# xinge008/SCDA

Hardware: AMD Instinct MI355X
Metric: images/sec (fwd+bwd) VGG16 Faster-RCNN+SCDA 512x1024 (higher is better)
Workload: dtype f32; 1 GPU; vgg16_FasterRCNN + 4-cluster SCDA, synthetic Cityscapes->Foggy 512x1024, batch=1/GPU (BASELINE.json configs[1]); 1 step = 1 source + 1 target image, 4 optimiser phases; gt_boxes=12, rois=512, clusters=4, recon=256, parallelism=dp1

## Files before the change

include/scda_ops.h:

```cpp
#ifndef SCDA_OPS_H
#define SCDA_OPS_H

#include <stddef.h>
#include <stdint.h>

#ifdef __cplusplus
extern "C" {
#endif

#define SCDA_OK 0
#define SCDA_EINVAL (-1)
#define SCDA_ELAUNCH (-2)
#define SCDA_ENODEV (-3)

int scda_version(void);
int scda_device_count(void);
const char *scda_last_error(void);

void scda_prof_enable(unsigned kernel_mask);
int scda_prof_num_kernels(void);
const char *scda_prof_kernel_name(int k);
int scda_prof_collect(long long *launches, double *ms, double *flops, double *bytes);
void scda_debug_last_plan(int *out4);
void scda_debug_plan_conv(int dir, int batch, int Cin, int IH, int IW, int Cout, int KH, int KW, int S, int P, int row_period,
// ... 142 lines not shown
size_t scda_eval_mark_duplicates_workspace_bytes(int n);
int scda_eval_mark_duplicates_hip(const int *image_ids, int n, void *ws, int *first, int *flags, int raise_on_duplicate, void *stream);
int scda_map_merge_duplicates_hip(const int *first, int n, int D, const int *box, const float *score, const int *cls, const int *rank,
                                  const int *kept, int *tp, int *flags, void *stream);

size_t scda_conv2d_workspace_bytes(int batch, int Cin, int IH, int IW, int Cout, int KH, int KW, int S, int P);
size_t scda_conv2d_packed_elems(int Cout, int Cin, int KH, int KW, int for_dgrad);
int scda_conv2d_pack_weight_hip(const float *w, float *out, int Cout, int Cin, int KH, int KW, int for_dgrad,
                                void *stream);
long long scda_conv2d_pack_tiles(int Cout, int Cin, int KH, int KW, int for_dgrad);
int scda_conv2d_pack_weights_batched_hip(const float *base, float *out, const long long *desc, int n, long long n_tiles,
                                         void *stream);
int scda_conv2d_fwd_hip(const float *x, const float *wp, const float *bias , float *y, int batch,
                        int Cin, int IH, int IW, int Cout, int KH, int KW, int S, int P, int row_period, int act, float slope,
                        void *ws, size_t ws_bytes, void *stream);
int scda_conv2d_dgrad_hip(const float *dy, const float *wt, float *dx, int batch, int Cin, int IH, int IW, int Cout,
                          int KH, int KW, int S, int P, int row_period, void *ws, size_t ws_bytes, void *stream);
int scda_conv2d_dgrad_act_hip(const float *dy, const float *wt, float *dx, int batch, int Cin, int IH, int IW, int Cout,
                              int KH, int KW, int S, int P, int row_period, const float *act_src, float act_slope, void *ws,
                              size_t ws_bytes, void *stream);
int scda_conv2d_dgrad_small_cin_hip(const float *dy, const float *w, float *dx, int batch, int Cin, int IH, int IW, int Cout,
                                    int KH, int KW, int S, int P, void *stream);
int scda_conv2d_wgrad_hip(const float *dy, const float *x, float *dw, int batch, int Cin, int IH, int IW, int Cout,
                          int KH, int KW, int S, int P, int row_period, int accumulate, void *ws, size_t ws_bytes, void *stream);
int scda_conv2d_wgrad_bias_fusable(int batch, int Cout, int OH, int OW, const float *dy);
int scda_conv2d_wgrad_bias_hip(const float *dy, const float *x, float *dw, float *db, int batch, int Cin, int IH, int IW,
                               int Cout, int KH, int KW, int S, int P, int row_period, int accumulate, int db_accumulate, void *ws,
                               size_t ws_bytes, void *stream);

int scda_conv2d_wino_supported(int batch, int C, int H, int W, int M);
// ... 120 lines not shown
```

scda_amd/autograd_ops.py:

```python
import os

import torch
from torch.autograd import Function

from . import native as N

ACT_NONE, ACT_RELU, ACT_LEAKY = N.ACT_NONE, N.ACT_RELU, N.ACT_LEAKY


from .probe import replay as _replay


def _c(t):
    return t if t.is_contiguous() else t.contiguous()


def _mask_src(ctx, y, kind="act"):
    r = _replay()
    if r is not None and any(ctx.needs_input_grad):
        return r.act(y)
    return y


def _sink(p):
# ... 40 lines not shown
            dw = None if sw is not None else dw
            db = None if sb is not None else db
        elif want_w:
            sink = _sink(ctx.w_ref)
            dw = N.conv2d_wgrad(dy, x, w.shape, stride, pad, out=sink, row_period=rp)
            if sink is not None:
                dw = None
        elif want_b:
            sink = _sink(ctx.bias_ref)
            db = N.bias_grad_nchw(dy, out=sink)
            if sink is not None:
                db = None
        return dx, dw, db, None, None, None, None, None, None


class ConvPoolFn(Function):

    @staticmethod
    def forward(ctx, x, w, b, slope, in_act):
        x = _c(x)
        if isinstance(w, torch.nn.Parameter):
            w._scda_wino_used = True
        y, idx = N.conv2d_wino_pool(x, N.conv2d_wino_pack(w, False), b, w.shape[0], ACT_RELU, slope)
        ctx.in_act = in_act
        ctx.has_bias = b is not None
        ctx.bias_ref, ctx.w_ref = b, w
        ctx.save_for_backward(x, w, idx, y)
        return y

    @staticmethod
# ... 435 lines not shown
class GlobalAvgPoolFn(Function):
    @staticmethod
    def forward(ctx, x):
        ctx.xshape = tuple(x.shape)
        return N.gap_fwd(_c(x))

    @staticmethod
    def backward(ctx, dy):
        return N.gap_bwd(_c(dy), ctx.xshape)


def conv2d(x, w, b=None, stride=1, padding=0, act=ACT_NONE, slope=0.01, fuse=(None, False), row_period=0):
    return Conv2dFn.apply(x, w, b, stride, padding, act, slope, fuse, row_period)


def linear(x, w, b=None, act=ACT_NONE, defer_act_bwd=False):
    return LinearFn.apply(x, w, b, act, defer_act_bwd)


def adversarial_loss(groups, scale=1.0):
    k = len(groups)
    return AdvLossFn.apply(scale, k, *[g[0] for g in groups], *[g[1] for g in groups], *[g[2] for g in groups])


def cross_entropy(logits, targets, ignore_index=-100):
    return SoftmaxCEFn.apply(logits, targets, ignore_index)


def smooth_l1_sum(pred, mask, target, sigma=3.0, scale=1.0):
    return SmoothL1Fn.apply(pred, mask, target, sigma, scale)
# ... 13 lines not shown
```

scda_amd/csrc/conv_gemm.hip:

```cpp
#include <stdio.h>
#include <stdlib.h>
#include <string.h>

#include "launch_plan.h"
#include "mfma_tile.h"
#include "wino_pack.h"

namespace scda {

__device__ __forceinline__ void tile_coords(const int nx, const int ny, const int swz, int &tx, int &ty, int &tz) {
    const unsigned nwg = gridDim.x, id = blockIdx.x;
    unsigned L = id;
    if (swz) {
        const unsigned q = nwg >> 3, r = nwg & 7, xcd = id & 7;
        L = (xcd < r ? xcd * (q + 1) : r * (q + 1) + (xcd - r) * q) + (id >> 3);
    }
    if (swz & 2) {
        const unsigned per = (unsigned)nx * ny, z = L / per, r = L - z * per;
        const unsigned grp = r / (8u * nx), first = grp * 8u, gsz = min((unsigned)ny - first, 8u), rr = r - grp * 8u * nx;
        tz = (int)z;
        tx = (int)(rr / gsz);
        ty = (int)(first + rr - (unsigned)tx * gsz);
        return;
    }
// ... 1552 lines not shown
#pragma unroll
        for (int kw = 0; kw < 3; ++kw) {
            const int iy = py + kh - 1, ix = px + kw - 1;
            const bool ok = iy >= 0 && iy < H && ix >= 0 && ix < W;
#pragma unroll
            for (int c = 0; c < CIN; ++c) v[(kh * 3 + kw) * CIN + c] = ok ? xi[((size_t)c * H + iy) * W + ix] : 0.f;
        }
    float *yo = y + ((size_t)img * Cout * H + py) * W + px;
    for (int m = 0; m < Cout; ++m) {
        const float *wm = wk + m * (9 * CIN);
        float a = 0.f;
#pragma unroll
        for (int k = 0; k < 9 * CIN; ++k) a = fmaf(wm[k], v[k], a);
        if (bias) a += bias[m];
        yo[(size_t)m * H * W] = apply_act(a, act, slope);
    }
}

template <int KH, int KW>
__global__ __launch_bounds__(256) void conv_dgrad_small_cin_kernel(const float *__restrict__ dY, const float *__restrict__ W,
                                                                   float *__restrict__ dX, const int batch, const int Cin,
                                                                   const int IH, const int IW, const int Cout, const int OH,
                                                                   const int OW, const int S, const int P) {
    extern __shared__ __attribute__((aligned(16))) float wl[];
    constexpr int R = KH * KW;
    for (int i = threadIdx.x; i < Cout * R * 4; i += blockDim.x) {
        const int m = i & 3, r = (i >> 2) % R, co = (i >> 2) / R;
        wl[i] = m < Cin ? W[((size_t)co * Cin + m) * R + r] : 0.f;
    }
    __syncthreads();
// ... 342 lines not shown
    if (d.family == lp::FAM_SMALL_CIN) {
        const dim3 grid((unsigned)cdiv(IW, 256), (unsigned)IH, (unsigned)batch);
        note_plan(d);
        prof_begin(PK_CONV_GATHER, 2.0 * Cout * (double)g.N * g.K, st);
        if (Cin == 1) hipLaunchKernelGGL((conv3x3_small_cin_fwd_kernel<1>), grid, dim3(256), 0, st, x, w, bias, y, IH, IW, Cout, act, slope);
        else if (Cin == 2) hipLaunchKernelGGL((conv3x3_small_cin_fwd_kernel<2>), grid, dim3(256), 0, st, x, w, bias, y, IH, IW, Cout, act, slope);
        else if (Cin == 3) hipLaunchKernelGGL((conv3x3_small_cin_fwd_kernel<3>), grid, dim3(256), 0, st, x, w, bias, y, IH, IW, Cout, act, slope);
        else hipLaunchKernelGGL((conv3x3_small_cin_fwd_kernel<4>), grid, dim3(256), 0, st, x, w, bias, y, IH, IW, Cout, act, slope);
        prof_end(st);
        return launch_status("conv3x3_small_cin_fwd_kernel");
    }
    Epi e{y, nullptr, bias, 0, act, slope, 1, 0, nullptr, 0.f};
    if (KH == 7 && KW == 7 && S == 2)
        return launch_conv<7, 7, 2, false>(d, w, x, g, e, (float *)ws, st);
    CONV_DISPATCH(launch_conv, , false > (d, w, x, g, e, (float *)ws, st))
}

SCDA_API int scda_conv2d_dgrad_hip(const float *dy, const float *wt, float *dx, int batch, int Cin, int IH, int IW,
                                   int Cout, int KH, int KW, int S, int P, int row_period, void *ws, size_t ws_bytes, void *stream) {
    return scda_conv2d_dgrad_act_hip(dy, wt, dx, batch, Cin, IH, IW, Cout, KH, KW, S, P, row_period, nullptr, 0.f, ws, ws_bytes, stream);
}

SCDA_API int scda_conv2d_dgrad_act_hip(const float *dy, const float *wt, float *dx, int batch, int Cin, int IH, int IW,
                                       int Cout, int KH, int KW, int S, int P, int row_period_arg, const float *act_src, float act_slope,
                                       void *ws, size_t ws_bytes, void *stream) {
    const int row_period = take_row_period("scda_conv2d_dgrad_hip", row_period_arg, IH, KH, KW, S, P);
    if (row_period < 0) return SCDA_EINVAL;
    if (!dy || !wt || !dx || batch <= 0) { set_error("scda_conv2d_dgrad_hip: bad arguments"); return SCDA_EINVAL; }
    const lp::ConvShape c{batch, Cin, IH, IW, Cout, KH, KW, S, P, row_period};
    const int OH = c.OH(), OW = c.OW();
// ... 177 lines not shown
```

scda_amd/csrc/launch_plan.h:

```cpp
#ifndef SCDA_LAUNCH_PLAN_H
#define SCDA_LAUNCH_PLAN_H

#include <stddef.h>
#include <stdio.h>
#include <stdlib.h>
#include <string.h>

#include <algorithm>
#include <vector>

namespace scda {
namespace lp {

constexpr int BK = 16;
constexpr int X9_BM = 256, X9_BN = 128;

static inline int cdiv(long long a, long long b) { return (int)((a + b - 1) / b); }
static inline int conv_out_dim(int in, int k, int s, int p) { return (in + 2 * p - k) / s + 1; }
static inline int conv_packed_mpad(int M) { return M <= 64 ? 64 : (M + 127) / 128 * 128; }

struct ForcedPlan { bool set; int bm, bn, splits; };
struct PlanEnv {
    ForcedPlan force;
    bool allow_bm64;
// ... 254 lines not shown
    d.nx = cdiv(N, d.bn); d.ny = cdiv(M, d.bm);
    d.swz = 1;
    if (d.parity) {
        d.nc = c.batch * (PH / 2) * (PW / 2);
        d.ncp = cdiv(d.nc, d.bn) * d.bn;
        d.nx = 4 * (d.ncp / d.bn);
        d.splits = fit_splits(std::max(1, std::min(plan.splits, (CB / BK) * taps)), M, N, ws_bytes);
    } else if (grouped_tile_order(d.nx, d.ny, M, K)) {
        d.swz |= 2;
    }
    d.grid = d.nx * d.ny * d.splits;
    d.reduce = d.splits > 1;
    return d;
}

static LaunchDecision decide_wgrad(const ConvShape &c, bool dy_aligned, bool aligned, bool fused_bias, size_t ws_bytes, int n_cu, const PlanEnv &env) {
    const int OH = c.OH(), OW = c.OW();
    const int M = c.Cout, N = c.Cin * c.KH * c.KW, K = c.batch * OH * OW;
    if (c.gemm_1x1() && !fused_bias && conv1x1_takes_x9(aligned, M, N, K, K, K, 0, 0, env)) return decide_gemm_x9(M, N, K, N, ws_bytes, n_cu, env);
    const bool small = M <= 64;
    const bool fits_2g = (long long)c.Cout * OH * OW * 4 < (1LL << 31) && (long long)c.Cin * c.IH * c.IW * 4 < (1LL << 31);
    const bool glds = dy_aligned && ((OH * OW) % BK) == 0 && fits_2g;
    TileRules r{};
    r.bm = small ? 64 : 128;
    r.allow64 = N <= 64; r.allow128 = !r.allow64; r.must_split = true; r.k_granule = 32;
    r.allow_bm256 = glds && r.allow128 && (M % 256) == 0;
    r.bn32 = (glds && M <= 32 && r.allow128) ? 128 : 0;
    LaunchPlan plan = plan_tiles(M, N, K, r, ws_bytes, env);
    if (r.bn32 && !env.force.set) plan.bm = 32;
    LaunchDecision d{};
// ... 181 lines not shown
```

scda_amd/dropin/_impl/rpn_head.py:

```python
import torch.nn as nn

from scda_amd import layers as L
from scda_amd.autograd_ops import ACT_RELU


class NaiveRpnHead(nn.Module):
    def __init__(self, inplanes, num_classes, num_anchors):
        super().__init__()
        self.num_classes = num_classes
        self.num_anchors = num_anchors
        self.conv3x3 = L.Conv2d(inplanes, 512, kernel_size=3, stride=1, padding=1, fused_act=ACT_RELU)
        self.relu3x3 = L.FusedAct("ReLU")
        self.conv_cls = L.Conv2d(512, num_anchors * num_classes, kernel_size=1, stride=1)
        self.conv_loc = L.Conv2d(512, num_anchors * 4, kernel_size=1, stride=1)

    def forward(self, x):
        hidden = self.relu3x3(self.conv3x3(x))
        return self.conv_cls(hidden), self.conv_loc(hidden)
```

scda_amd/dropin/models/faster_rcnn/faster_rcnn_adver_expansion_reweight_cluster.py:

```python
import functools
import logging

import os
import torch
import torch.nn as nn

from scda_amd import autograd_ops as A
from scda_amd import layers as L
from scda_amd import native as N
from scda_amd._timing import mark
from scda_amd.dropin.functions.anchor_target import compute_anchor_targets
from scda_amd.dropin.functions.mask import compute_cluster_targets
from scda_amd.dropin.functions.predict_bbox import compute_predicted_bboxes
from scda_amd.dropin.functions.proposal_target import compute_proposal_targets
from scda_amd.dropin.functions.rpn_proposal import compute_rpn_proposals
from scda_amd.dropin.models.faster_rcnn.common_net import (INSResBlock, LeakyReLUConv2d, LeakyReLUConvTranspose2d_2, LinUnsRes_cluster2,
                                                           LinUnsRes_cluster, ResDis_cluster, gaussian_weights_init, pair_decoder_upsamples)

logger = logging.getLogger('global')


def smooth_l1_loss_with_sigma(pred, targets, sigma=3.0):
    return A.smooth_l1_sum(pred, None, targets.contiguous(), sigma, 1.0)

# ... 31 lines not shown
    nhwc = rpn_pred_cls.detach().permute(0, 2, 3, 1).contiguous()
    prob = N.row_softmax(nhwc.view(-1, 2)).view_as(nhwc)
    return prob.permute(0, 3, 1, 2)


class FasterRCNN_AdEx(nn.Module):
    def __init__(self, gan_model_flag):
        super().__init__()

    def feature_extractor(self, x):
        raise NotImplementedError

    def rpn(self, x):
        raise NotImplementedError

    def rcnn(self, x, rois):
        raise NotImplementedError

    def _add_rpn_loss(self, compute_anchor_targets_fn, rpn_pred_cls, rpn_pred_loc):
        cls_targets, loc_targets, loc_masks, loc_normalizer = compute_anchor_targets_fn(rpn_pred_loc.size())
        logits = rpn_pred_cls.permute(0, 2, 3, 1).contiguous().view(-1, 2)
        flat_t = cls_targets.permute(0, 2, 3, 1).contiguous().view(-1)
        rpn_loss_cls = A.cross_entropy(logits, flat_t, ignore_index=-1)
        rpn_loss_loc = A.smooth_l1_sum(rpn_pred_loc, loc_masks, loc_targets, 3.0, 1.0 / loc_normalizer)
        acc = accuracy(logits, flat_t)[0]
        return rpn_loss_cls, rpn_loss_loc, acc

    def _add_rcnn_loss(self, rcnn_pred_cls, rcnn_pred_loc, cls_targets, loc_targets, loc_weights):
        rcnn_loss_cls = A.cross_entropy(rcnn_pred_cls, cls_targets)
        rcnn_loss_loc = A.smooth_l1_sum(rcnn_pred_loc, loc_weights, loc_targets, 3.0, 1.0 / cls_targets.shape[0])
        acc = accuracy(rcnn_pred_cls, cls_targets)[0]
# ... 87 lines not shown
            hook(losses)
            mark('det_backward_enqueued')
        clu_fea, clu_ctr = compute_cluster_targets(rois, x_fea, N_cluster=input['cluster_num'], threshold=input['threshold'])
        mark('src_cluster')
        side = input.get('_side_stream')
        main = torch.cuda.current_stream(dev) if side is not None else None

        def target_branch():
            with torch.no_grad():
                proposals_t = fn['rpn_proposal_fn'](*tgt_host())
                outputs['num_proposals_target'] = int(proposals_t.shape[0])
                rois_t_host = proposals_t[0:512, :5].contiguous()
                rois_t = N.upload(rois_t_host, dev)
                rois_t._scda_host = rois_t_host.numpy()
                assert rois_t.shape[1] == 5
                x_fea_t, _, _ = self.rcnn(feat_t, rois_t)
                return (x_fea_t,) + compute_cluster_targets(rois_t, x_fea_t, N_cluster=input['cluster_num'],
                                                            threshold=input['threshold'])

        if side is None:
            x_fea_t, clu_fea_t, clu_ctr_t = target_branch()
        else:
            side.wait_event(ev_backbones)
            with torch.cuda.stream(side):
                x_fea_t, clu_fea_t, clu_ctr_t = target_branch()
            main.wait_stream(side)
            for t in (x_fea_t, clu_fea_t):
                t.record_stream(main)
        assert feat_t.size() == feat.size(), "gan_features does not match the backbone"
        mark('target_branch')

# ... 30 lines not shown
    def __init__(self, params):
        super().__init__()
        ch, cin, n_layer = params['ch'], params['input_dim_a'], params['n_layer']
        self.model_A = self._make_net(ch, cin, n_layer - 1)
        self.model_A.apply(gaussian_weights_init)
        self.model_B = self._make_net(ch, cin, n_layer - 1)
        self.model_B.apply(gaussian_weights_init)
        L.plan_act_fusion(self.model_A, self.model_B)

    def _make_net(self, ch, input_dim, n_layer):
        seq = [LeakyReLUConv2d(input_dim, ch, kernel_size=3, stride=2, padding=1)]
        for _ in range(n_layer):
            seq.append(LeakyReLUConv2d(ch, ch * 2, kernel_size=3, stride=2, padding=1))
            ch *= 2
        seq.append(L.Conv2d(ch, 1, kernel_size=1, stride=1, padding=0))
        return nn.Sequential(*seq)

    def forward(self, x_aa, x_bb):
        a, b = _two_branches(self, lambda: self.model_A(x_aa), lambda: self.model_B(x_bb))
        return a.view(a.size(0), -1), b.view(b.size(0), -1)


class GAN_dis_AE_patch(nn.Module):

    def __init__(self, params=None):
        super().__init__()
        if params:
            self.n_in, self.n_out, clusters = params['n_in'], params['n_out'], params['cluster_num']
        else:
            self.n_in, self.n_out, clusters = 128, 256, 4
# ... 45 lines not shown
```

scda_amd/dropin/models/faster_rcnn/vgg_adver_expansion_cluster.py:

```python
import math

import torch.nn as nn

from scda_amd import layers as L
from scda_amd.autograd_ops import ACT_NONE, ACT_RELU
from scda_amd.dropin.extensions import RoIPool
from scda_amd.dropin.models.faster_rcnn.faster_rcnn_adver_expansion_reweight_cluster import FasterRCNN_AdEx
from scda_amd.dropin.models.head import NaiveRpnHead

__all__ = ['VGG', 'vgg16', 'vgg16_bn']

cfg = {
    'A': [64, 'M', 128, 'M', 256, 256, 'M', 512, 512, 'M', 512, 512, 'M'],
    'B': [64, 64, 'M', 128, 128, 'M', 256, 256, 'M', 512, 512, 'M', 512, 512, 'M'],
    'D': [64, 64, 'M', 128, 128, 'M', 256, 256, 256, 'M', 512, 512, 512, 'M', 512, 512, 512, 'M'],
    'E': [64, 64, 'M', 128, 128, 'M', 256, 256, 256, 256, 'M', 512, 512, 512, 512, 'M', 512, 512, 512, 512, 'M'],
}


def make_layers(plan, batch_norm=False):
    seq, cin = [], 3
    for v in plan:
        if v == 'M':
            seq.append(L.MaxPool2x2())
# ... 17 lines not shown
        self.roipooling = RoIPool(7, 7, 1.0 / cfg['anchor_stride'])
        self.classifier = nn.Sequential(
            L.Linear(512 * 7 * 7, 4096, fused_act=ACT_RELU), L.FusedAct("ReLU"), L.Dropout(),
            L.Linear(4096, 4096, fused_act=ACT_RELU), L.FusedAct("ReLU"), L.Dropout())
        self.fc_rcnn_cls = L.Linear(4096, cfg['num_classes'])
        self.fc_rcnn_loc = L.Linear(4096, cfg['num_classes'] * 4)
        L.plan_act_fusion(self.features, self.classifier)
        self._initialize_weights()

    def feature_extractor(self, x):
        return self.features(x)

    def rpn(self, x):
        return self.rpn_head(x)

    def rcnn(self, x, rois):
        assert rois.shape[1] == 5
        pooled = self.roipooling(x, rois)
        hook = getattr(self, '_head_grad_hook', None)
        if hook is not None and pooled.requires_grad:
            pooled.register_hook(lambda g: hook())
        x_fea = self.classifier(pooled.view(pooled.size(0), -1))
        return x_fea, self.fc_rcnn_cls(x_fea), self.fc_rcnn_loc(x_fea)

    def _initialize_weights(self):
        for m in self.modules():
            if isinstance(m, nn.Conv2d):
                fan = m.kernel_size[0] * m.kernel_size[1] * m.out_channels
                m.weight.data.normal_(0, math.sqrt(2. / fan))
                if m.bias is not None:
                    m.bias.data.zero_()
            elif isinstance(m, nn.BatchNorm2d):
                m.weight.data.fill_(1)
                m.bias.data.zero_()
            elif isinstance(m, nn.Linear):
                m.weight.data.normal_(0, 0.01)
                m.bias.data.zero_()
# ... 15 lines not shown
```

scda_amd/dropin/models/mask_rcnn/resnet.py:

```python
import math
import os

import torch
import torch.nn as nn

from scda_amd import autograd_ops as A
from scda_amd import layers as L
from scda_amd import native as N
from scda_amd.autograd_ops import ACT_NONE, ACT_RELU
from scda_amd.dropin.extensions._roi_align.modules.roi_align import RoIAlignAvg
from scda_amd.dropin.extensions import RoIPool
from scda_amd.dropin.models.faster_rcnn.faster_rcnn_adver_expansion_reweight_cluster import FasterRCNN_AdEx
from scda_amd.dropin.models.head import NaiveRpnHead

__all__ = ['ResNet', 'Bottleneck', 'resnet50', 'resnet101']


def _frozen(conv, bn):
    return (not bn.training and not conv.weight.requires_grad and not bn.weight.requires_grad and bn.running_mean is not None
            and conv.bias is None and not os.environ.get("SCDA_RESNET_NO_FOLD"))


def folded_conv_bn(x, conv, bn, act):
    key = tuple(t._version for t in (conv.weight, bn.weight, bn.bias, bn.running_mean, bn.running_var)) + (conv.weight.data_ptr(),)
# ... 113 lines not shown
    def _fix_layer(self, layer_num):
        for mod in [self.conv1, self.bn1] + [self.layer1, self.layer2, self.layer3, self.layer4][:layer_num]:
            for p in mod.parameters():
                p.requires_grad = False

    def feature_extractor(self, x):
        if _frozen(self.conv1, self.bn1):
            x = self.maxpool(folded_conv_bn(x, self.conv1, self.bn1, ACT_RELU))
        else:
            x = self.maxpool(self.bn1(self.conv1(x)))
        return self.layer3(self.layer2(self.layer1(x)))

    def rpn(self, x):
        return self.rpn_head(x)

    def rcnn(self, x, rois):
        assert rois.shape[1] == 5
        R = rois.shape[0]
        tall = (self.tall_head and isinstance(self.roipooling, RoIAlignAvg) and R > 0 and (R * 49) % 16 == 0
                and not os.environ.get("SCDA_RESNET_HEAD_NCHW"))
        self.roipooling.channel_major = tall
        for m in self._head_convs3x3:
            m.row_period = 7 if tall else 0
        x = self.roipooling(x, rois)
        if not tall:
            x = self.layer4(x)
            x_fea = self.avgpool(x).view(x.size(0), -1)
        else:
            C = x.shape[0]
            x = self.layer4(x.view(1, C, R * 7, 7))
            x_fea = self.avgpool(x.view(x.shape[1], R, 7, 7)).t().contiguous()
        return x_fea, self.fc_rcnn_cls(x_fea), self.fc_rcnn_loc(x_fea)


    def mask_predictor(self, x, rois):
        assert rois.shape[1] == 5
        R = rois.shape[0]
        tall = self.tall_head and R > 0 and R % 4 == 0 and not os.environ.get("SCDA_RESNET_HEAD_NCHW")
        self.mask_roipooling.channel_major = tall
        for m in self.mask_head.modules():
            if isinstance(m, L.Conv2d) and m.kernel_size == (3, 3):
                m.row_period = 14 if tall else 0
        x = self.mask_roipooling(x, rois)
        if not tall:
            return self.mask_head(x)
        y = self.mask_head(x.view(1, x.shape[0], R * 14, 14))
# ... 39 lines not shown
```

scda_amd/layers.py:

```python

import os
import weakref

import torch
import torch.nn as nn

from . import autograd_ops as A
from . import native as N
from . import probe as P


class FusedProducer:
    _consumer_ref = None
    _fusion_off_switch = None

    def hand_over_to(self, consumer):
        self._consumer_ref = weakref.ref(consumer)
        consumer._producer = weakref.ref(self)

    def fused_consumer(self):
        consumer = self._consumer_ref() if self._consumer_ref is not None else None
        if consumer is None or consumer._producer is None or consumer._producer() is not self:
            return None
        consumer._announced = None
# ... 39 lines not shown
        super().__init__(*args, **kw)
        if self.groups != 1 or self.dilation != (1, 1) or self.padding_mode != "zeros":
            raise NotImplementedError("scda_amd.Conv2d: groups/dilation/padding_mode are not part of the SCDA path")
        if self.stride[0] != self.stride[1] or self.padding[0] != self.padding[1]:
            raise NotImplementedError("scda_amd.Conv2d: anisotropic stride/padding")
        self.fused_act = fused_act
        self.slope = slope
        self.input_act = None
        self.defer_act_bwd = False
        self.row_period = 0

    @property
    def pool_next(self):
        return self._consumer_ref is not None

    def forward(self, x):
        pool = self.fused_consumer()
        if pool is not None and P.replay() is None and self.fused_act == A.ACT_RELU and self.defer_act_bwd:
            B, Cin, IH, IW = x.shape
            if x.is_cuda and N.conv_pool_fusable(B, Cin, IH, IW, self.out_channels, self.kernel_size[0], self.kernel_size[1],
                                                 self.stride[0], self.padding[0], self.row_period):
                y = A.ConvPoolFn.apply(x, self.weight, self.bias, self.slope, self.input_act)
                pool.announce(tuple(y.shape))
                return y
        return A.conv2d(x, self.weight, self.bias, self.stride[0], self.padding[0], self.fused_act, self.slope,
                        (self.input_act, self.defer_act_bwd), self.row_period)

    def extra_repr(self):
        s = super().extra_repr()
        return s + (f", fused_act={self.fused_act}" if self.fused_act else "")

# ... 239 lines not shown
```

scda_amd/native.py:

```python
import ctypes
import os
import re
import weakref

import torch

_HERE = os.path.dirname(os.path.abspath(__file__))
LIB_PATH = os.environ.get("SCDA_OPS_LIB") or os.path.join(_HERE, "libscda_ops.so")
HEADER_PATH = os.path.join(os.path.dirname(_HERE), "include", "scda_ops.h")

_lib = None


class ScdaNativeError(RuntimeError):
    pass


C_SCALARS = {"int": ctypes.c_int, "unsigned": ctypes.c_uint, "float": ctypes.c_float, "double": ctypes.c_double,
             "long long": ctypes.c_longlong, "size_t": ctypes.c_size_t, "uint64_t": ctypes.c_uint64}
C_RETURNS = dict(C_SCALARS, **{"void": None, "const char *": ctypes.c_char_p})


def parse_header(text):
    text = re.sub(r"/\*.*?\*/", " ", text, flags=re.S)
# ... 1003 lines not shown
    if bias is not None:
        _req(bias, "bias")
    B, Cin, IH, IW = x.shape
    Cout, Cin2, KH, KW = w.shape
    if Cin2 != Cin:
        raise ValueError(f"conv2d: input has {Cin} channels, weight expects {Cin2}")
    OH = (IH + 2 * pad - KH) // stride + 1
    OW = (IW + 2 * pad - KW) // stride + 1
    use_wino = wino_ok(B, Cin, IH, IW, Cout, KH, KW, stride, pad, row_period)
    if isinstance(w, torch.nn.Parameter):
        w._scda_wino_used = use_wino
    if use_wino:
        return conv2d_wino(x, conv2d_wino_pack(w, False), bias, Cout, act, slope, row_period=row_period)
    wp = conv2d_pack_weight(w, False)
    y = torch.empty(B, Cout, OH, OW, dtype=torch.float32, device=x.device)
    ws, n = _conv_ws(B, Cin, IH, IW, Cout, KH, KW, stride, pad, x.device)
    _check(lib().scda_conv2d_fwd_hip(_p(x), _p(wp), _p(bias), _p(y), B, Cin, IH, IW, Cout, KH, KW, stride, pad, row_period, act, slope,
                                     _p(ws), n, _stream()), "scda_conv2d_fwd_hip")
    return y


def conv2d_dgrad(dy, w, x_shape, stride, pad, act_src=None, act_slope=0.0, row_period=0):
    _req(dy, "dy"); _req(w, "w")
    B, Cin, IH, IW = x_shape
    Cout, _, KH, KW = w.shape
    if act_src is not None:
        _req(act_src, "act_src")
        if tuple(act_src.shape) != tuple(x_shape):
            raise ValueError("act_src must have the shape of the conv input")
    if _route(1, B, Cin, IH, IW, Cout, KH, KW, stride, pad, row_period)[0]:
# ... 541 lines not shown

PLAN_FIELDS = ("family", "x9_stream", "bm", "bn", "splits", "k_per_split", "nx", "ny", "grid", "swz", "parity", "nc", "ncp", "wbk",
               "reduce", "x9_r")


def plan_conv(direction, batch, cin, ih, iw, cout, k, stride, pad, row_period=0, aligned=True, ws_bytes=None):
    L = lib()
    if ws_bytes is None:
        ws_bytes = L.scda_conv2d_workspace_bytes(batch, cin, ih, iw, cout, k, k, stride, pad)
    out = (ctypes.c_int * 16)()
    L.scda_debug_plan_conv(("fwd", "dgrad", "wgrad", "wgrad_bias").index(direction), batch, cin, ih, iw, cout, k, k, stride, pad,
                           row_period, int(aligned), ws_bytes, out)
    return dict(zip(PLAN_FIELDS, out))


def plan_gemm(M, N, K, lda, ldb, trans_a=False, trans_b=False, aligned=True, ws_bytes=None, ldc=None):
    if ws_bytes is None:
        ws_bytes = max(16 * M * N * 4, 2 * 256 * 256 * 128 * 4)
    out = (ctypes.c_int * 16)()
    lib().scda_debug_plan_gemm(M, N, K, lda, ldb, N if ldc is None else ldc, int(trans_a), int(trans_b), int(aligned), ws_bytes, out)
    return dict(zip(PLAN_FIELDS, out))


WINO_PLAN_FIELDS = ("mb", "pixel_major", "gm", "splits", "slabs_per_split", "per_xcd", "n_wg", "persist", "epi")
WINO_WGRAD_PLAN_FIELDS = ("n_slab", "splits", "slabs_per_split", "splits_per_xcd", "order", "grid")


def plan_wino(kind, batch, cin, ih, iw, cout, row_period=0, ws_bytes=None):
    L = lib()
    if ws_bytes is None:
# ... 72 lines not shown
```

Baseline: 112.6 images/s.

## Add direct small-Cin stride-2 stem conv, thin 1x1 sibling head kernels, skip unused RCNN heads

Adds a direct per-pixel kernel for 3x3 stride-2 convolutions with at most four input channels, replacing the im2col/GEMM path for wide outputs. Adds thin_map forward and dgrad kernels that compute one or two narrow 1x1 convolution heads in a single pass over the input; these now serve discriminator final layers flagged thin_head. It also lets the target-domain RCNN call skip the classification and regression heads when only features are needed. The aim is to cut launch overhead and poor GEMM utilisation on tiny-N or tiny-K shapes, at the price of extra code paths and new dispatch heuristics.

```diff
diff --git a/include/scda_ops.h b/include/scda_ops.h
--- a/include/scda_ops.h
+++ b/include/scda_ops.h
@@ -180,6 +180,14 @@
 int scda_conv2d_fwd_hip(const float *x, const float *wp, const float *bias , float *y, int batch,
                         int Cin, int IH, int IW, int Cout, int KH, int KW, int S, int P, int row_period, int act, float slope,
                         void *ws, size_t ws_bytes, void *stream);
+int scda_conv2d_small_cin_s2_fwd_hip(const float *x, const float *wp, const float *bias , float *y, int batch,
+                                     int Cin, int IH, int IW, int Cout, int act, float slope, void *stream);
+void scda_debug_plan_stem_s2(int batch, int Cin, int IH, int IW, int Cout, int KH, int KW, int S, int P, int row_period, int *out6);
+int scda_thin_map_fwd_hip(const float *x, const float *w0, const float *b0, float *y0, int n0, const float *w1, const float *b1,
+                          float *y1, int n1, int batch, int C, int HW, int act, float slope, void *stream);
+int scda_thin_map_dgrad_hip(const float *dy0, const float *w0, int n0, const float *dy1, const float *w1, int n1, float *dx,
+                            int batch, int C, int HW, const float *act_src, float act_slope, void *stream);
+void scda_debug_plan_thin_map(int batch, int C, int HW, int n0, int n1, int *out9);
 int scda_conv2d_dgrad_hip(const float *dy, const float *wt, float *dx, int batch, int Cin, int IH, int IW, int Cout,
                           int KH, int KW, int S, int P, int row_period, void *ws, size_t ws_bytes, void *stream);
 int scda_conv2d_dgrad_act_hip(const float *dy, const float *wt, float *dx, int batch, int Cin, int IH, int IW, int Cout,
diff --git a/scda_amd/autograd_ops.py b/scda_amd/autograd_ops.py
--- a/scda_amd/autograd_ops.py
+++ b/scda_amd/autograd_ops.py
@@ -78,6 +78,50 @@
         return dx, dw, db, None, None, None, None, None, None
 
 
+class SiblingConv1x1Fn(Function):
+
+    @staticmethod
+    def forward(ctx, x, in_act, *wb):
+        x = _c(x)
+        ws, bs = list(wb[0::2]), list(wb[1::2])
+        ys = N.thin_map_fwd(x, ws, bs)
+        ctx.in_act = in_act if _replay() is None else None
+        ctx.w_refs, ctx.bias_refs = ws, bs
+        ctx.save_for_backward(x, *ws)
+        return tuple(ys)
+
+    @staticmethod
+    def backward(ctx, *dys):
+        x, *ws = ctx.saved_tensors
+        dys = [_c(dy) for dy in dys]
+        in_act = ctx.in_act
+        grads = [None, None]
+        if ctx.needs_input_grad[0]:
+            grads[0] = N.thin_map_dgrad(dys, ws, x.shape, act_src=x if in_act is not None else None,
+                                        act_slope=0.0 if in_act is None or in_act[0] == ACT_RELU else in_act[1])
+        for i, (dy, w) in enumerate(zip(dys, ws)):
+            dw = db = None
+            bias = ctx.bias_refs[i]
+            want_w, want_b = ctx.needs_input_grad[2 + 2 * i], bias is not None and ctx.needs_input_grad[3 + 2 * i]
+            if want_w and want_b:
+                sw, sb = _sink(ctx.w_refs[i]), _sink(bias)
+                dw, db = N.conv2d_wgrad_bias(dy, x, w.shape, 1, 0, out=sw, db_out=sb)
+                dw = None if sw is not None else dw
+                db = None if sb is not None else db
+            elif want_w:
+                sink = _sink(ctx.w_refs[i])
+                dw = N.conv2d_wgrad(dy, x, w.shape, 1, 0, out=sink)
+                if sink is not None:
+                    dw = None
+            elif want_b:
+                sink = _sink(bias)
+                db = N.bias_grad_nchw(dy, out=sink)
+                if sink is not None:
+                    db = None
+            grads += [dw, db]
+        return tuple(grads)
+
+
 class ConvPoolFn(Function):
 
     @staticmethod
@@ -543,6 +587,10 @@
     return Conv2dFn.apply(x, w, b, stride, padding, act, slope, fuse, row_period)
 
 
+def sibling_conv1x1(x, heads, input_act=None):
+    return SiblingConv1x1Fn.apply(x, input_act, *[t for wb in heads for t in wb])
+
+
 def linear(x, w, b=None, act=ACT_NONE, defer_act_bwd=False):
     return LinearFn.apply(x, w, b, act, defer_act_bwd)
 
diff --git a/scda_amd/csrc/conv_gemm.hip b/scda_amd/csrc/conv_gemm.hip
--- a/scda_amd/csrc/conv_gemm.hip
+++ b/scda_amd/csrc/conv_gemm.hip
@@ -1590,6 +1590,152 @@
         for (int k = 0; k < 9 * CIN; ++k) a = fmaf(wm[k], v[k], a);
         if (bias) a += bias[m];
         yo[(size_t)m * H * W] = apply_act(a, act, slope);
+    }
+}
+
+template <int CIN>
+__global__ __launch_bounds__(256) void conv3x3s2_small_cin_fwd_kernel(const float *__restrict__ x, const float *__restrict__ wk,
+                                                                      const float *__restrict__ bias, float *__restrict__ y, const int H,
+                                                                      const int W, const int OH, const int OW, const int Cout,
+                                                                      const int cout_per, const int act, const float slope) {
+    const int p = blockIdx.x * 256 + threadIdx.x, img = blockIdx.z;
+    if (p >= OH * OW) return;
+    const int py = p / OW, px = p - py * OW;
+    const float *xi = x + (size_t)img * CIN * H * W;
+    float v[9 * CIN];
+#pragma unroll
+    for (int kh = 0; kh < 3; ++kh)
+#pragma unroll
+        for (int kw = 0; kw < 3; ++kw) {
+            const int iy = 2 * py + kh - 1, ix = 2 * px + kw - 1;
+            const bool ok = iy >= 0 && iy < H && ix >= 0 && ix < W;
+#pragma unroll
+            for (int c = 0; c < CIN; ++c) v[(kh * 3 + kw) * CIN + c] = ok ? xi[((size_t)c * H + iy) * W + ix] : 0.f;
+        }
+    const size_t plane = (size_t)OH * OW;
+    float *yo = y + (size_t)img * Cout * plane + p;
+    const int m0 = blockIdx.y * cout_per, m1 = min(Cout, m0 + cout_per);
+    for (int m = m0; m < m1; ++m) {
+        const float *wm = wk + m * (9 * CIN);
+        float a = 0.f;
+#pragma unroll
+        for (int k = 0; k < 9 * CIN; ++k) a = fmaf(wm[k], v[k], a);
+        if (bias) a += bias[m];
+        yo[(size_t)m * plane] = apply_act(a, act, slope);
+    }
+}
+
+struct ThinSiblings {
+    const float *w[2];
+    const float *bias[2];
+    float *y[2];
+    int n[2];
+};
+
+constexpr int THIN_NT = lp::THIN_NT, THIN_NW = lp::THIN_NW, THIN_CT = lp::THIN_CT, THIN_DW = lp::THIN_DW;
+
+__global__ __launch_bounds__(THIN_NW * 64) void thin_map_fwd_kernel(const float *__restrict__ x, const ThinSiblings sb, const int C,
+                                                                    const int HW, const int chunks0, const int ch_per_wave,
+                                                                    const int act, const float slope) {
+    __shared__ float red[THIN_NW][THIN_NT][64];
+    const int lane = threadIdx.x & 63, wave = __builtin_amdgcn_readfirstlane(threadIdx.x >> 6);
+    const int s = blockIdx.y >= (unsigned)chunks0 ? 1 : 0;
+    const int n0 = (blockIdx.y - (s ? chunks0 : 0)) * THIN_NT, N = sb.n[s];
+    const int p = blockIdx.x * 64 + lane, pc = min(p, HW - 1);
+    const float *xp = x + (size_t)blockIdx.z * C * HW + pc;
+    const float *wr[THIN_NT];
+#pragma unroll
+    for (int j = 0; j < THIN_NT; ++j) wr[j] = sb.w[s] + (size_t)min(n0 + j, N - 1) * C;
+    float a[THIN_NT];
+#pragma unroll
+    for (int j = 0; j < THIN_NT; ++j) a[j] = 0.f;
+    const int c0 = wave * ch_per_wave, c1 = min(C, c0 + ch_per_wave);
+    int c = c0;
+    for (; c + 8 <= c1; c += 8) {
+        float v[8];
+#pragma unroll
+        for (int u = 0; u < 8; ++u) v[u] = xp[(size_t)(c + u) * HW];
+#pragma unroll
+        for (int u = 0; u < 8; ++u)
+#pragma unroll
+            for (int j = 0; j < THIN_NT; ++j) a[j] = fmaf(wr[j][c + u], v[u], a[j]);
+    }
+    for (; c < c1; ++c) {
+        const float v = xp[(size_t)c * HW];
+#pragma unroll
+        for (int j = 0; j < THIN_NT; ++j) a[j] = fmaf(wr[j][c], v, a[j]);
+    }
+#pragma unroll
+    for (int j = 0; j < THIN_NT; ++j) red[wave][j][lane] = a[j];
+    __syncthreads();
+    const int n = n0 + wave;
+    if (n >= N || p >= HW) return;
+    float t = red[0][wave][lane];
+#pragma unroll
+    for (int k = 1; k < THIN_NW; ++k) t += red[k][wave][lane];
+    if (sb.bias[s]) t += sb.bias[s][n];
+    sb.y[s][((size_t)blockIdx.z * N + n) * HW + p] = apply_act(t, act, slope);
+}
+
+__global__ __launch_bounds__(THIN_DW * 64) void thin_map_dgrad_kernel(const ThinSiblings sb, float *__restrict__ dx, const int C,
+                                                                      const int HW, const float *__restrict__ act_src,
+                                                                      const float act_slope) {
+    constexpr int CB = THIN_DW * THIN_CT, DR = 32;
+    __shared__ __attribute__((aligned(16))) float wl[DR][CB];
+    const int lane = threadIdx.x & 63, wave = __builtin_amdgcn_readfirstlane(threadIdx.x >> 6);
+    const int cb0 = blockIdx.y * CB, c0 = cb0 + wave * THIN_CT;
+    const int p = blockIdx.x * 64 + lane, pc = min(p, HW - 1);
+    float a[THIN_CT];
+#pragma unroll
+    for (int j = 0; j < THIN_CT; ++j) a[j] = 0.f;
+    for (int s = 0; s < 2; ++s) {
+        const int N = sb.n[s];
+        if (N <= 0) continue;
+        const float *g = sb.y[s] + (size_t)blockIdx.z * N * HW + pc;
+        const float *w = sb.w[s];
+        for (int n0 = 0; n0 < N; n0 += DR) {
+            const int nr = min(DR, N - n0);
+            __syncthreads();
+            for (int i = threadIdx.x; i < nr * CB; i += THIN_DW * 64) {
+                const int r = i / CB, c = cb0 + i % CB;
+                wl[r][i % CB] = c < C ? w[(size_t)(n0 + r) * C + c] : 0.f;
+            }
+            __syncthreads();
+            const float4 *wr = reinterpret_cast<const float4 *>(&wl[0][wave * THIN_CT]);
+            int r = 0;
+            for (; r + 4 <= nr; r += 4) {
+                float v[4];
+#pragma unroll
+                for (int u = 0; u < 4; ++u) v[u] = g[(size_t)(n0 + r + u) * HW];
+#pragma unroll
+                for (int u = 0; u < 4; ++u)
+#pragma unroll
+                    for (int q = 0; q < THIN_CT / 4; ++q) {
+                        const float4 w4 = wr[(r + u) * (CB / 4) + q];
+                        a[4 * q] = fmaf(w4.x, v[u], a[4 * q]); a[4 * q + 1] = fmaf(w4.y, v[u], a[4 * q + 1]);
+                        a[4 * q + 2] = fmaf(w4.z, v[u], a[4 * q + 2]); a[4 * q + 3] = fmaf(w4.w, v[u], a[4 * q + 3]);
+                    }
+            }
+            for (; r < nr; ++r) {
+                const float v = g[(size_t)(n0 + r) * HW];
+#pragma unroll
+                for (int q = 0; q < THIN_CT / 4; ++q) {
+                    const float4 w4 = wr[r * (CB / 4) + q];
+                    a[4 * q] = fmaf(w4.x, v, a[4 * q]); a[4 * q + 1] = fmaf(w4.y, v, a[4 * q + 1]);
+                    a[4 * q + 2] = fmaf(w4.z, v, a[4 * q + 2]); a[4 * q + 3] = fmaf(w4.w, v, a[4 * q + 3]);
+                }
+            }
+        }
+    }
+    if (p >= HW) return;
+#pragma unroll
+    for (int j = 0; j < THIN_CT; ++j) {
+        if (c0 + j < C) {
+            const size_t i = ((size_t)blockIdx.z * C + c0 + j) * HW + p;
+            float t = a[j];
+            if (act_src) t *= act_src[i] > 0.f ? 1.f : act_slope;
+            dx[i] = t;
+        }
     }
 }
 
@@ -1962,6 +2108,58 @@
     if (KH == 7 && KW == 7 && S == 2)
         return launch_conv<7, 7, 2, false>(d, w, x, g, e, (float *)ws, st);
     CONV_DISPATCH(launch_conv, , false > (d, w, x, g, e, (float *)ws, st))
+}
+
+SCDA_API int scda_conv2d_small_cin_s2_fwd_hip(const float *x, const float *wk, const float *bias, float *y, int batch, int Cin, int IH,
+                                              int IW, int Cout, int act, float slope, void *stream) {
+    const lp::ConvShape c{batch, Cin, IH, IW, Cout, 3, 3, 2, 1, 0};
+    const lp::StemDecision d = lp::decide_stem_s2(c);
+    if (!x || !wk || !y || !d.legal) { set_error("scda_conv2d_small_cin_s2_fwd_hip: bad arguments"); return SCDA_EINVAL; }
+    const int OH = c.OH(), OW = c.OW();
+    const dim3 grid((unsigned)d.px_blocks, (unsigned)d.chunks, (unsigned)batch);
+    hipStream_t st = as_stream(stream);
+    prof_begin(PK_CONV_GATHER, 2.0 * Cout * (double)batch * OH * OW * 9 * Cin, st);
+#define STEM_S2_LAUNCH(CIN_) hipLaunchKernelGGL((conv3x3s2_small_cin_fwd_kernel<CIN_>), grid, dim3(256), 0, st, x, wk, bias, y, IH, IW, OH, OW, Cout, d.cout_per, act, slope)
+    if (Cin == 1) STEM_S2_LAUNCH(1);
+    else if (Cin == 2) STEM_S2_LAUNCH(2);
+    else if (Cin == 3) STEM_S2_LAUNCH(3);
+    else STEM_S2_LAUNCH(4);
+#undef STEM_S2_LAUNCH
+    prof_end(st);
+    return launch_status("conv3x3s2_small_cin_fwd_kernel");
+}
+
+SCDA_API void scda_debug_plan_stem_s2(int batch, int Cin, int IH, int IW, int Cout, int KH, int KW, int S, int P, int row_period, int *out6) {
+    const lp::StemDecision d = lp::decide_stem_s2(lp::ConvShape{batch, Cin, IH, IW, Cout, KH, KW, S, P, row_period});
+    static_assert(sizeof(lp::StemDecision) == 6 * sizeof(int), "scda_ops.h documents 6 ints");
+    memcpy(out6, &d, sizeof d);
+}
+
+SCDA_API int scda_thin_map_fwd_hip(const float *x, const float *w0, const float *b0, float *y0, int n0, const float *w1, const float *b1,
+                                   float *y1, int n1, int batch, int C, int HW, int act, float slope, void *stream) {
+    static_assert(THIN_NT == THIN_NW, "thin_map_fwd_kernel sums one output per thread");
+    const lp::ThinMapDecision d = lp::decide_thin_map(batch, C, HW, n0, n1);
+    if (!x || !w0 || !y0 || !d.legal || (n1 > 0 && (!w1 || !y1))) { set_error("scda_thin_map_fwd_hip: bad arguments"); return SCDA_EINVAL; }
+    const ThinSiblings sb{{w0, n1 > 0 ? w1 : nullptr}, {b0, n1 > 0 ? b1 : nullptr}, {y0, n1 > 0 ? y1 : nullptr}, {n0, n1}};
+    hipLaunchKernelGGL(thin_map_fwd_kernel, dim3((unsigned)d.px_blocks, (unsigned)(d.chunks0 + d.chunks1), (unsigned)batch), dim3(THIN_NW * 64), 0,
+                       as_stream(stream), x, sb, C, HW, d.chunks0, d.ch_per_wave, act, slope);
+    return launch_status("thin_map_fwd_kernel");
+}
+
+SCDA_API int scda_thin_map_dgrad_hip(const float *dy0, const float *w0, int n0, const float *dy1, const float *w1, int n1, float *dx,
+                                     int batch, int C, int HW, const float *act_src, float act_slope, void *stream) {
+    const lp::ThinMapDecision d = lp::decide_thin_map(batch, C, HW, n0, n1);
+    if (!dy0 || !w0 || !dx || !d.legal || (n1 > 0 && (!w1 || !dy1))) { set_error("scda_thin_map_dgrad_hip: bad arguments"); return SCDA_EINVAL; }
+    const ThinSiblings sb{{w0, n1 > 0 ? w1 : nullptr}, {nullptr, nullptr}, {const_cast<float *>(dy0), n1 > 0 ? const_cast<float *>(dy1) : nullptr}, {n0, n1}};
+    hipLaunchKernelGGL(thin_map_dgrad_kernel, dim3((unsigned)d.px_blocks, (unsigned)d.dgrad_cblocks, (unsigned)batch), dim3(THIN_DW * 64), 0,
+                       as_stream(stream), sb, dx, C, HW, act_src, act_slope);
+    return launch_status("thin_map_dgrad_kernel");
+}
+
+SCDA_API void scda_debug_plan_thin_map(int batch, int C, int HW, int n0, int n1, int *out9) {
+    const lp::ThinMapDecision d = lp::decide_thin_map(batch, C, HW, n0, n1);
+    static_assert(sizeof(lp::ThinMapDecision) == 9 * sizeof(int), "scda_ops.h documents 9 ints");
+    memcpy(out9, &d, sizeof d);
 }
 
 SCDA_API int scda_conv2d_dgrad_hip(const float *dy, const float *wt, float *dx, int batch, int Cin, int IH, int IW,
diff --git a/scda_amd/csrc/launch_plan.h b/scda_amd/csrc/launch_plan.h
--- a/scda_amd/csrc/launch_plan.h
+++ b/scda_amd/csrc/launch_plan.h
@@ -292,6 +292,60 @@
     return d;
 }
 
+struct StemDecision {
+    int legal, wanted;
+    int px_blocks;
+    int chunks, cout_per;
+    int grid;
+};
+
+static StemDecision decide_stem_s2(const ConvShape &c) {
+    StemDecision d{};
+    d.legal = c.KH == 3 && c.KW == 3 && c.S == 2 && c.P == 1 && c.Cin >= 1 && c.Cin <= 4 && c.Cout >= 1 && c.batch >= 1 && c.batch <= 65535 &&
+              c.row_period == 0 && c.IH >= 1 && c.IW >= 1 && (long long)c.OH() * c.OW() < (1LL << 31) - 256;
+    if (!d.legal) return d;
+    const int OH = c.OH(), OW = c.OW();
+    d.wanted = OW >= 64;
+    d.px_blocks = cdiv(OH * OW, 256);
+    const long long blocks = (long long)d.px_blocks * c.batch;
+    const int most = cdiv(c.Cout, 8);
+    const int chunks = (int)std::max<long long>(1, std::min<long long>(most, 1024 / blocks));
+    d.cout_per = cdiv(c.Cout, chunks);
+    d.chunks = cdiv(c.Cout, d.cout_per);
+    d.grid = (int)std::min<long long>(blocks * d.chunks, 0x7fffffff);
+    return d;
+}
+
+constexpr int THIN_NT = 8;
+constexpr int THIN_NW = 8;
+constexpr int THIN_CT = 16;
+constexpr int THIN_DW = 4;
+
+struct ThinMapDecision {
+    int legal, wanted;
+    int px_blocks;
+    int chunks0, chunks1;
+    int ch_per_wave;
+    int grid;
+    int dgrad_cblocks, dgrad_grid;
+};
+
+static ThinMapDecision decide_thin_map(int batch, int C, long long HW, int n0, int n1) {
+    ThinMapDecision d{};
+    d.legal = batch >= 1 && batch <= 65535 && C >= 1 && HW >= 1 && HW < (1LL << 31) - 64 && n0 >= 1 && n1 >= 0 && n0 <= 65536 && n1 <= 65536 &&
+              C <= 65536 * 16;
+    if (!d.legal) return d;
+    d.wanted = n0 + n1 <= 128;
+    d.px_blocks = cdiv((int)HW, 64);
+    d.chunks0 = cdiv(n0, THIN_NT);
+    d.chunks1 = cdiv(n1, THIN_NT);
+    d.ch_per_wave = cdiv(C, THIN_NW);
+    d.grid = (int)std::min<long long>((long long)d.px_blocks * (d.chunks0 + d.chunks1) * batch, 0x7fffffff);
+    d.dgrad_cblocks = cdiv(C, THIN_DW * THIN_CT);
+    d.dgrad_grid = (int)std::min<long long>((long long)d.px_blocks * d.dgrad_cblocks * batch, 0x7fffffff);
+    return d;
+}
+
 static LaunchDecision decide_wgrad(const ConvShape &c, bool dy_aligned, bool aligned, bool fused_bias, size_t ws_bytes, int n_cu, const PlanEnv &env) {
     const int OH = c.OH(), OW = c.OW();
     const int M = c.Cout, N = c.Cin * c.KH * c.KW, K = c.batch * OH * OW;
diff --git a/scda_amd/dropin/_impl/rpn_head.py b/scda_amd/dropin/_impl/rpn_head.py
--- a/scda_amd/dropin/_impl/rpn_head.py
+++ b/scda_amd/dropin/_impl/rpn_head.py
@@ -1,7 +1,8 @@
 import torch.nn as nn
 
 from scda_amd import layers as L
-from scda_amd.autograd_ops import ACT_RELU
+from scda_amd import native as N
+from scda_amd.autograd_ops import ACT_RELU, sibling_conv1x1
 
 
 class NaiveRpnHead(nn.Module):
@@ -16,4 +17,7 @@
 
     def forward(self, x):
         hidden = self.relu3x3(self.conv3x3(x))
+        if hidden.is_cuda and N.plan_thin_map(hidden.shape[0], hidden.shape[1], hidden.shape[2] * hidden.shape[3],
+                                              self.conv_cls.out_channels, self.conv_loc.out_channels)["wanted"]:
+            return sibling_conv1x1(hidden, [(self.conv_cls.weight, self.conv_cls.bias), (self.conv_loc.weight, self.conv_loc.bias)])
         return self.conv_cls(hidden), self.conv_loc(hidden)
diff --git a/scda_amd/dropin/models/faster_rcnn/faster_rcnn_adver_expansion_reweight_cluster.py b/scda_amd/dropin/models/faster_rcnn/faster_rcnn_adver_expansion_reweight_cluster.py
--- a/scda_amd/dropin/models/faster_rcnn/faster_rcnn_adver_expansion_reweight_cluster.py
+++ b/scda_amd/dropin/models/faster_rcnn/faster_rcnn_adver_expansion_reweight_cluster.py
@@ -69,7 +69,7 @@
     def rpn(self, x):
         raise NotImplementedError
 
-    def rcnn(self, x, rois):
+    def rcnn(self, x, rois, heads=True):
         raise NotImplementedError
 
     def _add_rpn_loss(self, compute_anchor_targets_fn, rpn_pred_cls, rpn_pred_loc):
@@ -187,7 +187,7 @@
                 rois_t = N.upload(rois_t_host, dev)
                 rois_t._scda_host = rois_t_host.numpy()
                 assert rois_t.shape[1] == 5
-                x_fea_t, _, _ = self.rcnn(feat_t, rois_t)
+                x_fea_t, _, _ = self.rcnn(feat_t, rois_t, heads=False)
                 return (x_fea_t,) + compute_cluster_targets(rois_t, x_fea_t, N_cluster=input['cluster_num'],
                                                             threshold=input['threshold'])
 
@@ -248,6 +248,7 @@
             seq.append(LeakyReLUConv2d(ch, ch * 2, kernel_size=3, stride=2, padding=1))
             ch *= 2
         seq.append(L.Conv2d(ch, 1, kernel_size=1, stride=1, padding=0))
+        seq[-1].thin_head = True
         return nn.Sequential(*seq)
 
     def forward(self, x_aa, x_bb):
diff --git a/scda_amd/dropin/models/faster_rcnn/vgg_adver_expansion_cluster.py b/scda_amd/dropin/models/faster_rcnn/vgg_adver_expansion_cluster.py
--- a/scda_amd/dropin/models/faster_rcnn/vgg_adver_expansion_cluster.py
+++ b/scda_amd/dropin/models/faster_rcnn/vgg_adver_expansion_cluster.py
@@ -55,13 +55,15 @@
     def rpn(self, x):
         return self.rpn_head(x)
 
-    def rcnn(self, x, rois):
+    def rcnn(self, x, rois, heads=True):
         assert rois.shape[1] == 5
         pooled = self.roipooling(x, rois)
         hook = getattr(self, '_head_grad_hook', None)
         if hook is not None and pooled.requires_grad:
             pooled.register_hook(lambda g: hook())
         x_fea = self.classifier(pooled.view(pooled.size(0), -1))
+        if not heads:
+            return x_fea, None, None
         return x_fea, self.fc_rcnn_cls(x_fea), self.fc_rcnn_loc(x_fea)
 
     def _initialize_weights(self):
diff --git a/scda_amd/dropin/models/mask_rcnn/resnet.py b/scda_amd/dropin/models/mask_rcnn/resnet.py
--- a/scda_amd/dropin/models/mask_rcnn/resnet.py
+++ b/scda_amd/dropin/models/mask_rcnn/resnet.py
@@ -151,7 +151,7 @@
     def rpn(self, x):
         return self.rpn_head(x)
 
-    def rcnn(self, x, rois):
+    def rcnn(self, x, rois, heads=True):
         assert rois.shape[1] == 5
         R = rois.shape[0]
         tall = (self.tall_head and isinstance(self.roipooling, RoIAlignAvg) and R > 0 and (R * 49) % 16 == 0
@@ -167,6 +167,8 @@
             C = x.shape[0]
             x = self.layer4(x.view(1, C, R * 7, 7))
             x_fea = self.avgpool(x.view(x.shape[1], R, 7, 7)).t().contiguous()
+        if not heads:
+            return x_fea, None, None
         return x_fea, self.fc_rcnn_cls(x_fea), self.fc_rcnn_loc(x_fea)
 
 
diff --git a/scda_amd/layers.py b/scda_amd/layers.py
--- a/scda_amd/layers.py
+++ b/scda_amd/layers.py
@@ -77,7 +77,13 @@
     def pool_next(self):
         return self._consumer_ref is not None
 
-    def forward(self, x):
+    thin_head = False
+
+    def forward(self, x):
+        if self.thin_head and x.is_cuda:
+            if self.kernel_size != (1, 1) or self.stride != (1, 1) or self.padding != (0, 0) or self.fused_act != A.ACT_NONE:
+                raise NotImplementedError("scda_amd.Conv2d: thin_head is a plain 1x1 convolution")
+            return A.sibling_conv1x1(x, [(self.weight, self.bias)], self.input_act)[0]
         pool = self.fused_consumer()
         if pool is not None and P.replay() is None and self.fused_act == A.ACT_RELU and self.defer_act_bwd:
             B, Cin, IH, IW = x.shape
diff --git a/scda_amd/native.py b/scda_amd/native.py
--- a/scda_amd/native.py
+++ b/scda_amd/native.py
@@ -1041,6 +1041,10 @@
         return conv2d_wino(x, conv2d_wino_pack(w, False), bias, Cout, act, slope, row_period=row_period)
     wp = conv2d_pack_weight(w, False)
     y = torch.empty(B, Cout, OH, OW, dtype=torch.float32, device=x.device)
+    if Cin <= 4 and stride == 2 and KH == KW and plan_stem_s2(B, Cin, IH, IW, Cout, KH, stride, pad, row_period)["wanted"]:
+        _check(lib().scda_conv2d_small_cin_s2_fwd_hip(_p(x), _p(wp), _p(bias), _p(y), B, Cin, IH, IW, Cout, act, slope, _stream()),
+               "scda_conv2d_small_cin_s2_fwd_hip")
+        return y
     ws, n = _conv_ws(B, Cin, IH, IW, Cout, KH, KW, stride, pad, x.device)
     _check(lib().scda_conv2d_fwd_hip(_p(x), _p(wp), _p(bias), _p(y), B, Cin, IH, IW, Cout, KH, KW, stride, pad, row_period, act, slope,
                                      _p(ws), n, _stream()), "scda_conv2d_fwd_hip")
@@ -1612,6 +1616,97 @@
     return dict(zip(PLAN_FIELDS, out))
 
 
+STEM_PLAN_FIELDS = ("legal", "wanted", "px_blocks", "chunks", "cout_per", "grid")
+
+
+def plan_stem_s2(batch, cin, ih, iw, cout, k, stride, pad, row_period=0):
+    out = (ctypes.c_int * 6)()
+    lib().scda_debug_plan_stem_s2(batch, cin, ih, iw, cout, k, k, stride, pad, row_period, out)
+    return dict(zip(STEM_PLAN_FIELDS, out))
+
+
+def conv2d_small_cin_s2_fwd(x, w, bias, act=ACT_NONE, slope=0.01, out=None):
+    _req(x, "x"); _req(w, "w")
+    if bias is not None:
+        _req(bias, "bias")
+    B, Cin, IH, IW = x.shape
+    Cout, Cin2, KH, KW = w.shape
+    if Cin2 != Cin or (KH, KW) != (3, 3):
+        raise ValueError("conv2d_small_cin_s2_fwd: a 3x3 weight on the input's channels")
+    shape = (B, Cout, (IH - 1) // 2 + 1, (IW - 1) // 2 + 1)
+    if out is None:
+        y = torch.empty(shape, dtype=torch.float32, device=x.device)
+    else:
+        _req(out, "out")
+        if tuple(out.shape) != shape:
+            raise ValueError("conv2d_small_cin_s2_fwd: out must be %s" % (shape,))
+        y = out
+    _check(lib().scda_conv2d_small_cin_s2_fwd_hip(_p(x), _p(conv2d_pack_weight(w, False)), _p(bias), _p(y), B, Cin, IH, IW, Cout, act, slope,
+                                                  _stream()), "scda_conv2d_small_cin_s2_fwd_hip")
+    return y
+
+
+THIN_MAP_PLAN_FIELDS = ("legal", "wanted", "px_blocks", "chunks0", "chunks1", "ch_per_wave", "grid", "dgrad_cblocks", "dgrad_grid")
+
+
+def plan_thin_map(batch, c, hw, n0, n1=0):
+    out = (ctypes.c_int * 9)()
+    lib().scda_debug_plan_thin_map(batch, c, hw, n0, n1, out)
+    return dict(zip(THIN_MAP_PLAN_FIELDS, out))
+
+
+def _thin_siblings(who, x_shape, ws):
+    B, C, H, W = x_shape
+    if not 1 <= len(ws) <= 2:
+        raise ValueError("%s: one or two siblings" % who)
+    for w in ws:
+        _req(w, "w")
+        if tuple(w.shape[1:]) != (C, 1, 1):
+            raise ValueError("%s: every sibling is a 1x1 weight on the input's %d channels, got %s" % (who, C, tuple(w.shape)))
+    return B, C, H, W
+
+
+def thin_map_fwd(x, ws, biases, act=ACT_NONE, slope=0.01, out=None):
+    _req(x, "x")
+    B, C, H, W = _thin_siblings("thin_map_fwd", x.shape, ws)
+    for b in biases:
+        if b is not None:
+            _req(b, "bias")
+    ys = out if out is not None else [torch.empty(B, w.shape[0], H, W, dtype=torch.float32, device=x.device) for w in ws]
+    for y, w in zip(ys, ws):
+        _req(y, "out")
+        if tuple(y.shape) != (B, w.shape[0], H, W):
+            raise ValueError("thin_map_fwd: out of %s for a sibling of %d channels" % (tuple(y.shape), w.shape[0]))
+    two = len(ws) == 2
+    _check(lib().scda_thin_map_fwd_hip(_p(x), _p(ws[0]), _p(biases[0]), _p(ys[0]), ws[0].shape[0], _p(ws[1]) if two else None,
+                                       _p(biases[1]) if two else None, _p(ys[1]) if two else None, ws[1].shape[0] if two else 0,
+                                       B, C, H * W, act, slope, _stream()), "scda_thin_map_fwd_hip")
+    return list(ys)
+
+
+def thin_map_dgrad(dys, ws, x_shape, act_src=None, act_slope=0.0, out=None):
+    B, C, H, W = _thin_siblings("thin_map_dgrad", x_shape, ws)
+    for dy, w in zip(dys, ws):
+        _req(dy, "dy")
+        if tuple(dy.shape) != (B, w.shape[0], H, W):
+            raise ValueError("thin_map_dgrad: dy of %s for a sibling of %d channels" % (tuple(dy.shape), w.shape[0]))
+    if act_src is not None:
+        _req(act_src, "act_src")
+        if tuple(act_src.shape) != tuple(x_shape):
+            raise ValueError("act_src must have the shape of the heads' input")
+    if out is None:
+        out = torch.empty(B, C, H, W, dtype=torch.float32, device=dys[0].device)
+    else:
+        _req(out, "out")
+        if tuple(out.shape) != (B, C, H, W):
+            raise ValueError("thin_map_dgrad: out must be %s" % ((B, C, H, W),))
+    two = len(ws) == 2
+    _check(lib().scda_thin_map_dgrad_hip(_p(dys[0]), _p(ws[0]), ws[0].shape[0], _p(dys[1]) if two else None, _p(ws[1]) if two else None,
+                                         ws[1].shape[0] if two else 0, _p(out), B, C, H * W, _p(act_src), act_slope, _stream()),
+           "scda_thin_map_dgrad_hip")
+    return out
+
+
 def plan_gemm(M, N, K, lda, ldb, trans_a=False, trans_b=False, aligned=True, ws_bytes=None, ldc=None):
     if ws_bytes is None:
         ws_bytes = max(16 * M * N * 4, 2 * 256 * 256 * 128 * 4)
```

Result: slower. 109.0 images/s (-3.2%).
